# kazuto1011/dusty-gan

Measured on AMD Instinct MI355X. Metric: G+D train images/sec on 64x1024 LiDAR (steps/sec beside it), higher is better.
Workload: dtype bf16

## Files before the change

dusty_gan_amd/csrc/api.hip:

```cpp
#include "common.h"
#include "thin.h"

int dg_conv_direct_launch(const ConvP* p, hipStream_t stream);
int dg_lrelu_bits_launch(const ConvP* p, hipStream_t stream);
int dg_conv_mfma_launch(const ConvP* p, hipStream_t stream, int force, int fp32x3, int wg_cap, DgConvPlan* plan);
int dg_wgrad_mfma_dma_supported(const WgradP* p);
int dg_wgrad_mfma_dma_launch(const WgradP* p, int accumulate, int pairs, hipStream_t stream, DgWgradPlan* plan);
int dg_wgrad_mfma_dma_group_launch(const WgradP* items, int n, int pairs, int rounds, hipStream_t stream, DgWgradPlan* plans);
int dg_proj_stream_supported(const ConvP* p);
int dg_proj_stream_launch(const ConvP* p, hipStream_t stream, DgConvPlan* plan);
int dg_wgrad_mfma_ws_splits(const WgradP* p, int accumulate);
int dg_wgrad_direct_ws_splits(const WgradP* p);
int dg_wgrad_direct_launch(const WgradP* p, hipStream_t stream);
int dg_wgrad_mfma_launch(const WgradP* p, int accumulate, hipStream_t stream, int x3);

namespace {

enum ConvKernel { CONV_DIRECT, CONV_THIN, CONV_MFMA, CONV_PROJ_STREAM };

int select_conv(const DgConv* p, int force_flags, ConvKernel* k, ThinConvPick* thin, DgConvPlan* plan) {
  if (p && (p->mask_out || p->mask_in)) {
    if (p->mask_out && p->epi != EPI_LRELU) return DG_EINVAL;
    if (p->mask_in && p->epi != EPI_MASK) return DG_EINVAL;
    if (p->out_sn != 1 || p->N % 8 != 0 || p->out_sp % 8 != 0 || p->out_sb % 8 != 0) return DG_EUNSUPPORTED;
  }
  if (!p || !p->in || !p->out || !p->w) return DG_EINVAL;
  if (p->B <= 0 || p->K <= 0 || p->N <= 0) return DG_EINVAL;
  if (p->mode != MODE_GEMM && (p->Hc < 2 || p->Wc < 2)) return DG_EINVAL;
  if (p->epi == EPI_MASK && !p->aux) return DG_EINVAL;
  if (p->bias && p->bias_mod <= 0) return DG_EINVAL;
  if (p->dbias && p->bias_mod <= 0) return DG_EINVAL;
  if (plan) *plan = DgConvPlan{};
  const int force = force_flags & ~DG_FORCE_FP32X3;
  const bool mfma_ok = !p->nscale && dg_conv_mfma_supported(p), thin_ok = thin_conv_pick(p, thin) == DG_OK;
  const bool proj_ok = dg_proj_stream_supported(p);
  bool ok = true;
  if (force == DG_FORCE_AUTO) *k = proj_ok ? CONV_PROJ_STREAM : (mfma_ok ? CONV_MFMA : (thin_ok ? CONV_THIN : CONV_DIRECT));
  else if (force == DG_FORCE_PROJ_STREAM) *k = CONV_PROJ_STREAM, ok = proj_ok;
  else if (force == DG_FORCE_MFMA || force == DG_FORCE_LOCKSTEP || force == DG_FORCE_PINGPONG ||
           force == DG_FORCE_PINGPONG_SINGLE) *k = CONV_MFMA, ok = mfma_ok;
  else if (force == DG_FORCE_THIN) *k = CONV_THIN, ok = thin_ok;
  else *k = CONV_DIRECT;
  return ok ? DG_OK : DG_EUNSUPPORTED;
}

int conv_run(const DgConv* p, ConvKernel k, const ThinConvPick& thin, int force_flags, int wg_cap, hipStream_t s, DgConvPlan* plan) {
  if (k == CONV_PROJ_STREAM) return dg_proj_stream_launch(p, s, plan);
  if (k == CONV_MFMA)
    return dg_conv_mfma_launch(p, s, force_flags & ~DG_FORCE_FP32X3, (force_flags & DG_FORCE_FP32X3) ? 1 : 0, wg_cap, plan);
  if (!plan) return k == CONV_THIN ? thin_conv_launch(p, thin, s) : dg_conv_direct_launch(p, s);
  plan->family = k == CONV_THIN ? DG_CONV_FAMILY_THIN : DG_CONV_FAMILY_DIRECT;
  if (k == CONV_THIN)
    plan->thin_mfma = thin.thin_mfma, plan->mask_bits = thin.mask_bits, plan->dbias_rows = thin.dbias_rows, plan->sum_parts = thin.sum_parts;
  return DG_OK;
}

int conv_dispatch(const DgConv* p, int force_flags, int wg_cap, hipStream_t s, DgConvPlan* plan) {
  ConvKernel k;
  ThinConvPick thin;
  int rc = select_conv(p, force_flags, &k, &thin, plan);
  if (rc || plan || !p->mask_out) return rc ? rc : conv_run(p, k, thin, force_flags, wg_cap, s, plan);
  DgConvPlan pl{};
  rc = conv_run(p, k, thin, force_flags, wg_cap, nullptr, &pl);
  if (rc == DG_OK) rc = conv_run(p, k, thin, force_flags, wg_cap, s, nullptr);
// ... 2 lines not shown
}

struct WgradKernel {
  int variant;
  int pairs;
  int splits;
  long ws_floats;
  bool takes_gmod;
  bool zero_dw;
  ThinWgradPick thin;
};

int select_wgrad(const DgWgrad* p, int accumulate, int force_flags, WgradKernel* k) {
  if (!p || !p->a || !p->g || !p->dw) return DG_EINVAL;
  if (p->B <= 0 || p->Ci <= 0 || p->Co <= 0 || p->Hc <= 0 || p->Wc <= 0) return DG_EINVAL;
  const int force = force_flags & ~DG_FORCE_FP32X3;
  ThinWgradPick thin;
  const bool mfma_ok = dg_wgrad_mfma_supported(p), thin_ok = thin_wgrad_pick(p, &thin) == DG_OK;
  const bool pairs = force == DG_FORCE_WG_DMA_PAIRS || force == DG_FORCE_WG_DMA_NOPAIRS;
  *k = WgradKernel{};
  if ((force == DG_FORCE_AUTO || force == DG_FORCE_MFMA || pairs) && mfma_ok && dg_wgrad_mfma_dma_supported(p)) {
    k->variant = DG_WGRAD_VARIANT_DMA, k->takes_gmod = true;
    k->pairs = force == DG_FORCE_WG_DMA_PAIRS ? 1 : (force == DG_FORCE_WG_DMA_NOPAIRS ? 2 : 0);
    return DG_OK;
  }
  if (force == DG_FORCE_AUTO)
    k->variant = mfma_ok ? DG_WGRAD_VARIANT_MFMA : (thin_ok ? DG_WGRAD_VARIANT_THIN : DG_WGRAD_VARIANT_DIRECT);
  else if (force == DG_FORCE_MFMA || force == DG_FORCE_WG_REGSTAGED) k->variant = mfma_ok ? DG_WGRAD_VARIANT_MFMA : 0;
  else if (force == DG_FORCE_THIN) k->variant = thin_ok ? DG_WGRAD_VARIANT_THIN : 0;
  else if (!pairs) k->variant = DG_WGRAD_VARIANT_DIRECT;
  if (!k->variant) return DG_EUNSUPPORTED;
// ... 74 lines not shown
```

dusty_gan_amd/csrc/conv_mfma.hip:

```cpp
#include "mfma_common.h"

#ifndef DG_CONV_SETPRIO
#define DG_CONV_SETPRIO 1
#endif

template <typename T, int BM, int BN, int SB, int NS, bool X3 = false>
__global__ __launch_bounds__(256, 2) void conv_mfma_kernel(ConvP p, int tiles_n, int tiles_x, int dbg) {
  static_assert(!X3 || sizeof(T) == 4, "fp32x3: fp32 operands");
  constexpr int ES = sizeof(T);
  constexpr bool PRIO = DG_CONV_SETPRIO;
  constexpr int BK = SB / ES;
  constexpr int EPC = 16 / ES;
  constexpr int TM = BM / 64, TN = BN / 64;
  constexpr int RPI = 1024 / SB;
  constexpr int CPR = SB / 16;
  constexpr int KS = SB / 32;
  constexpr int STAGE = (BM + BN) * SB;
  constexpr int IA = BM / RPI / 4, IB = BN / RPI / 4;
  constexpr int IPT = IA + IB;
  __shared__ __attribute__((aligned(1024))) unsigned char lds[NS * STAGE];

  const int nwg = gridDim.x, id = blockIdx.x;
  const int q8 = nwg >> 3, r8 = nwg & 7, xcd = id & 7;
  const int logical = (xcd < r8 ? xcd * (q8 + 1) : r8 * (q8 + 1) + (xcd - r8) * q8) + (id >> 3);
// ... 289 lines not shown
  conv_mfma_kernel<T, BM, BN, 128, 2, X3><<<(unsigned)nwg, 256, 0, stream>>>(*p, tiles_n, tiles_x, 0);
  HIP_CHECK_RET(hipGetLastError());
  return DG_OK;
}

template <typename T, bool X3 = false>
static int launch_tiles(const ConvP* p, hipStream_t stream, DgConvPlan* plan) {
  const bool m128 = p->mode == MODE_GEMM ? false : (p->Wc % 128 == 0);
  const bool n128 = p->N % 128 == 0;
  if (m128 && n128) return launch_cfg<T, 128, 128, X3>(p, stream, plan);
  if (m128) return launch_cfg<T, 128, 64, X3>(p, stream, plan);
  if (n128) return launch_cfg<T, 64, 128, X3>(p, stream, plan);
  return launch_cfg<T, 64, 64, X3>(p, stream, plan);
}

int dg_conv_mfma_pp_launch(const ConvP* p, hipStream_t stream, int min_tiles, int wg_cap, DgConvPlan* plan, int dual);

extern "C" int dg_conv_mfma_supported(const ConvP* p) {
  if (p->in_dtype == DG_BF16X2 || p->out_dtype == DG_BF16X2 || p->w_dtype == DG_BF16X2) {
    DgConvPlan pl;
    return dg_conv_mfma_pp_launch(p, nullptr, 1, 0, &pl, 1) == DG_OK;
  }
  const int es = p->in_dtype == DG_BF16 ? 2 : 4;
  const int BK = 128 / es;
  if (p->in_dtype != p->out_dtype || p->in_dtype != p->w_dtype) return 0;
  if (p->K % BK != 0 || p->N % 64 != 0) return 0;
  if (p->in_sk != 1 || p->w_sk != 1 || p->out_sn != 1) return 0;
  if (p->mode == MODE_GEMM) return p->dbias == nullptr;
  if (!p->ring) return 0;
  if (p->Wc % 64 != 0) return 0;
  if (p->dbias && p->bias_mod < p->N) return 0;
  return 1;
}

int dg_conv_mfma_persist_launch_bf16(const ConvP* p, hipStream_t stream, int auto_rule, int wg_cap, DgConvPlan* plan);
int dg_conv_mfma_persist_launch_f32(const ConvP* p, hipStream_t stream, int auto_rule, int wg_cap, DgConvPlan* plan);

int dg_conv_mfma_launch(const ConvP* p, hipStream_t stream, int force, int fp32x3, int wg_cap, DgConvPlan* plan) {
  if (!dg_conv_mfma_supported(p)) return DG_EUNSUPPORTED;
  if (force == DG_FORCE_PINGPONG || force == DG_FORCE_PINGPONG_SINGLE)
    return (p->in_dtype == DG_BF16 || p->in_dtype == DG_BF16X2)
               ? dg_conv_mfma_pp_launch(p, stream, 1, wg_cap, plan, force == DG_FORCE_PINGPONG) : DG_EUNSUPPORTED;
  if (force == DG_FORCE_LOCKSTEP) {
    if (p->in_dtype == DG_BF16X2) return DG_EUNSUPPORTED;
    return p->in_dtype == DG_BF16 ? dg_conv_mfma_persist_launch_bf16(p, stream, 0, wg_cap, plan)
                                  : dg_conv_mfma_persist_launch_f32(p, stream, 0, wg_cap, plan);
  }
  if (p->in_dtype == DG_BF16X2) return dg_conv_mfma_pp_launch(p, stream, 1, wg_cap, plan, 1);
  if (p->in_dtype == DG_BF16) {
    const int rc = dg_conv_mfma_pp_launch(p, stream, 256, wg_cap, plan, 1);
    if (rc != DG_EUNSUPPORTED) return rc;
  }
  const bool x3 = p->in_dtype == DG_F32 && fp32x3;
  if (!x3) {
    const int rc = p->in_dtype == DG_BF16 ? dg_conv_mfma_persist_launch_bf16(p, stream, 1, wg_cap, plan)
                                          : dg_conv_mfma_persist_launch_f32(p, stream, 1, wg_cap, plan);
    if (rc != DG_EUNSUPPORTED) return rc;
  }
  if (x3) return launch_tiles<float, true>(p, stream, plan);
  return p->in_dtype == DG_BF16 ? launch_tiles<bf16>(p, stream, plan) : launch_tiles<float>(p, stream, plan);
}
```

dusty_gan_amd/csrc/conv_mfma_persist_impl.h:

```cpp
#pragma once
#include "mfma_common.h"

namespace persist {

template <typename T> struct StageWrite;
template <> struct StageWrite<bf16> {
  static __device__ __forceinline__ void put(unsigned addr, float v) {
    const bf16 h = (bf16)v;
    const unsigned bits = (unsigned)__builtin_bit_cast(unsigned short, h);
    asm volatile("ds_write_b16 %0, %1" ::"v"(addr), "v"(bits) : "memory");
  }
};
template <> struct StageWrite<float> {
  static __device__ __forceinline__ void put(unsigned addr, float v) {
    asm volatile("ds_write_b32 %0, %1" ::"v"(addr), "v"(v) : "memory");
  }
};

struct Tile {
  int nt, xt, px, Y, bt;
};

template <int MODE>
__device__ __forceinline__ bool next_tile(Tile& t, int tiles_n, int tiles_x, int rows) {
// ... 18 lines not shown
    int r, ky;
    if (dg_tap1d(MODE, adj, 0, Y, Hc, i, r, ky)) {
      list |= (unsigned long long)((r << 2) | ky) << (10 * n);
      ++n;
    }
  }
  return n;
}

#define DG_WAITV(n) asm volatile("s_waitcnt vmcnt(%0)" ::"n"(n) : "memory")

struct Geo {
  int tiles_n, tiles_x, ntiles;
  int SW, NSB, lsw;
  int dbg;
};

template <typename T, int BM, int BN, int WM, int WN, int SB, int NS, int MODE>
__global__ __launch_bounds__(64 * WM * WN, 1) void conv_kernel(ConvP p, Geo g) {
  constexpr int NWV = WM * WN;
  constexpr int ES = sizeof(T);
  constexpr int BK = SB / ES;
  constexpr int EPC = 16 / ES;
  constexpr int TM = BM / WM / 32, TN = BN / WN / 32;
  constexpr int RPI = 1024 / SB;
  constexpr int CPR = SB / 16;
  constexpr int KS = SB / 32;
  constexpr int STAGE = (BM + BN) * SB;
  constexpr int IA = BM / RPI / NWV, IB = BN / RPI / NWV;
  constexpr int IPT = IA + IB;
// ... 424 lines not shown
```

dusty_gan_amd/csrc/conv_mfma_pp.hip:

```cpp
#include "conv_mfma_persist_impl.h"

#include <type_traits>

namespace pp {

using persist::Geo;
using persist::Tile;

typedef __attribute__((ext_vector_type(4))) float f32x4_t;

#define PP_WAIT(vm) asm volatile("s_waitcnt vmcnt(%0) lgkmcnt(0)" ::"n"(vm) : "memory")

constexpr int NHT = 256;
struct HTab { unsigned long long e[NHT]; };

__device__ __forceinline__ unsigned long long pp_stamp() {
  unsigned long long t;
  __builtin_amdgcn_sched_barrier(0);
  asm volatile("s_memtime %0\n\ts_waitcnt lgkmcnt(0)" : "=s"(t)::"memory");
  __builtin_amdgcn_sched_barrier(0);
  return t;
}

template <int CTRL>
__device__ __forceinline__ float row_add(float v) {
  const int s = __builtin_amdgcn_update_dpp(0, __builtin_bit_cast(int, v), CTRL, 0xf, 0xf, false);
  return v + __builtin_bit_cast(float, s);
}

template <int BN, int MODE, bool MASK, bool DUAL = false, bool BITS = false, bool X2 = false>
__global__ __launch_bounds__(512, 2) void conv_pp_kernel(ConvP p, Geo g, HTab ht) {
  static_assert(MASK || !BITS, "BITS: a flavour of the EPI_MASK epilogue");
  static_assert(!X2 || !BITS, "X2: mask source = the saved activation's hi half");
  static_assert(!DUAL || (MODE == MODE_UP && BN == 128), "DUAL: both column parities of a 64-channel MODE_UP layer");
  constexpr int NCH = DUAL ? BN / 2 : BN;
  constexpr int BM = 256, NWV = 8, WN = 2;
  constexpr int SB = 128;
  constexpr int WC = BN / WN;
  constexpr int TM = 4, TN = WC / 16;
  constexpr int CPL = 4 * TN;
  constexpr int IMG_ROWS = 264;
  constexpr int AIMG = IMG_ROWS * SB;
  constexpr int BT = BN * SB;
  constexpr int PSTAGE = AIMG + 2 * BT;
  constexpr int NPS = 2;
  constexpr int IA = 4, IB = BN / 8 / NWV;
  constexpr int NST = TM * CPL * 2 / 16;
// ... 11 lines not shown
  constexpr int dbg = DG_PP_DIAG;
#else
  constexpr int dbg = 0;
#endif

  const int G = gridDim.x;
  const int q8 = G >> 3, r8 = G & 7, xcd = blockIdx.x & 7;
  const int gi0 = xcd < r8 ? xcd * (q8 + 1) : r8 * (q8 + 1) + (xcd - r8) * q8;
  const int nwx = q8 + (xcd < r8 ? 1 : 0);
  const int tq = g.ntiles / G, tr = g.ntiles % G;
  const int xs = gi0 * tq + (gi0 < tr ? gi0 : tr);
  const int xe = (gi0 + nwx) * tq + (gi0 + nwx < tr ? gi0 + nwx : tr);
  const int t0 = xs + (int)(blockIdx.x >> 3);
  const int tcount = t0 < xe ? (xe - t0 + nwx - 1) / nwx : 0;
  if (tcount == 0) {
    if (MASK && p.dbias && p.dbias_part)
      for (int n = threadIdx.x; n < p.N; n += 64 * NWV) p.dbias_part[(long)blockIdx.x * p.N + n] = 0.f;
    return;
  }

  const unsigned long long tk0 = (dbg & 8) ? pp_stamp() : 0ull;
  const unsigned long long tr0 = (dbg & 8) ? __builtin_amdgcn_s_memrealtime() : 0ull;
  const int tid = threadIdx.x;
  const int wave = __builtin_amdgcn_readfirstlane(tid >> 6), lane = tid & 63;
  const int KC = p.K / 64;
  const int Ws = MODE == MODE_S2 ? 2 * p.Wc : p.Wc, cmul = MODE == MODE_S2 ? 2 : 1;
  const int Wo = MODE == MODE_S2 ? p.Wc : 2 * p.Wc;
  const int rows = MODE == MODE_S2 ? p.Hc : 2 * p.Hc;
  const int tiles_n = g.tiles_n, tiles_x = g.tiles_x;

  auto tile_at = [&](int t) {
// ... 17 lines not shown
    dstep.xt = r % tiles_x; r /= tiles_x;
    dstep.px = 0;
    if (MODE == MODE_UP && !DUAL) { dstep.px = r & 1; r >>= 1; }
    dstep.Y = r % rows; dstep.bt = r / rows;
    dstep.nt = __builtin_amdgcn_readfirstlane(dstep.nt); dstep.xt = __builtin_amdgcn_readfirstlane(dstep.xt);
    dstep.px = __builtin_amdgcn_readfirstlane(dstep.px); dstep.Y = __builtin_amdgcn_readfirstlane(dstep.Y);
    dstep.bt = __builtin_amdgcn_readfirstlane(dstep.bt);
  }
  auto tile_next = [&](Tile& t) __attribute__((always_inline)) {
    int c;
    t.nt += dstep.nt; c = t.nt >= tiles_n; if (c) t.nt -= tiles_n;
    t.xt += dstep.xt + c; c = t.xt >= tiles_x; if (c) t.xt -= tiles_x;
    if (MODE == MODE_UP && !DUAL) { t.px += dstep.px + c; c = t.px >> 1; t.px &= 1; }
    t.Y += dstep.Y + c; c = t.Y >= rows; if (c) t.Y -= rows;
    t.bt += dstep.bt + c;
  };

  const bf16* in = (const bf16*)p.in;
  const bf16* w = (const bf16*)p.w;
  const int lrow = lane >> 3, pos = lane & 7;
  auto swzA = [](int row) { return ((row >> 1) & 3) << 1; };
  auto swzB = [](int row) { return ((row >> 1) & 1) | (((row / CPL) & 3) << 1); };

  unsigned voffA[NPAIR][IA + 1], voffB[IB];
  int colA[IA + 1];
  unsigned sampA[IA + 1];
  {
    const int pitch = g.SW + (DUAL ? 2 : 1);
#pragma unroll
    for (int u = 0; u <= IA; ++u) {
// ... 96 lines not shown
      for (int i = 0; i < TM; ++i) {
        const char* src = mb + (long)i * px_b;
        if (CPL == 16) asm volatile("global_load_ushort %0, %1, %2" : "=v"(mbits[i]) : "v"(pix_off_m), "s"(src) : "memory");
        else asm volatile("global_load_ubyte %0, %1, %2" : "=v"(mbits[i]) : "v"(pix_off_m), "s"(src) : "memory");
      }
    } else {
      const char* ab = (const char*)((const bf16*)p.aux + tile_off(t));
#pragma unroll
      for (int i = 0; i < TM; ++i) {
        const char* src = ab + (long)(i * 16) * px_b;
        asm volatile("global_load_dwordx4 %0, %1, %2" : "=v"(axr[(NST / TM) * i]) : "v"(pix_off), "s"(src) : "memory");
        if (NST / TM == 2) asm volatile("global_load_dwordx4 %0, %1, %2 offset:16" : "=v"(axr[2 * i + 1]) : "v"(pix_off), "s"(src) : "memory");
      }
    }
  };
  auto flush_db = [&](float (&dbacc)[CPL], int nt) __attribute__((always_inline)) {
#pragma unroll
    for (int c = 0; c < CPL; ++c) dbacc[c] = row_add<0xB1>(dbacc[c]);
#pragma unroll
    for (int c = 0; c < CPL; ++c) dbacc[c] = row_add<0x4E>(dbacc[c]);
#pragma unroll
    for (int c = 0; c < CPL; ++c) dbacc[c] = row_add<0x124>(dbacc[c]);
#pragma unroll
    for (int c = 0; c < CPL; ++c) dbacc[c] = row_add<0x128>(dbacc[c]);
    if (a16 == 0) {
      const unsigned ad = sdbw0 + (unsigned)(nt * NCH * 4) + lane_c0 * 4;
#pragma unroll
      for (int c = 0; c < CPL; ++c) asm volatile("ds_add_f32 %0, %1 offset:%2" ::"v"(ad), "v"(dbacc[c]), "n"(c * 4) : "memory");
    }
  };
  auto epilogue = [&](const Tile& t) __attribute__((always_inline)) {
    char* ob = (char*)(out + tile_off(t));
    if (MASK && !BITS) {
#pragma unroll
      for (int i = 0; i < NST; ++i) asm volatile("" : "+v"(axr[i]));
    }
    if (BITS) {
#pragma unroll
      for (int i = 0; i < TM; ++i) asm volatile("" : "+v"(mbits[i]));
// ... 100 lines not shown
          }
          continue;
        }
        if (h == 0 && i > 0) store_row(i - 1);
        asm volatile("ds_write_b128 %0, %1" ::"v"(scr_w ^ (unsigned)(h << 4)), "v"(pk) : "memory");
      }
      if (STRIP) {
        asm volatile("s_waitcnt lgkmcnt(0)" ::: "memory");
#pragma unroll
        for (int h = 0; h < NRD; ++h)
          asm volatile("ds_read_b128 %0, %1 offset:%2" : "=v"(rd[h]) : "v"(scr_r), "n"(h * 1024) : "memory");
      }
      __builtin_amdgcn_sched_barrier(0);
    }
    if (STRIP) store_row(TM - 1);
    if (want_db) flush_db(dbacc, t.nt);
    zero_acc();
  };

  const bool stamps = (dbg & 8) != 0;
  unsigned long long tsum[6] = {0, 0, 0, 0, 0, 0};
  unsigned long long tend = 0, tkf = 0;

  if (wave >= 4) __builtin_amdgcn_s_barrier();
  unsigned so_c = PSTAGE, so_i = 0;
  bool pending = false;
  bool warm = true;
  Tile tprev = first;
  const long tap_b = (long)p.w_st * 2;
  const unsigned spb = (unsigned)p.in_sp * 2u;

// ... 94 lines not shown
      if (stamps) t4 = pp_stamp();
      if (ISS || t == 0 || wave < 4) __builtin_amdgcn_s_barrier();
      if (stamps) {
        t5 = pp_stamp();
        tsum[0] += t1 - t0; tsum[1] += t2 - t1; tsum[2] += t3 - t2; tsum[3] += t4 - t3; tsum[4] += t5 - t4;
        tend = t5;
      }
    };
    step(std::integral_constant<int, 0>{});
    step(std::integral_constant<int, 1>{});
    const unsigned sw_ = so_c; so_c = so_i; so_i = sw_;
  };

  Tile ti = first;
  for (int c = 0; c < tcount; ++c) {
    unsigned long long hl;
    int nh;
    {
      const unsigned long long e = ht.e[ti.Y];
      nh = (int)(e >> 60) & 7;
      hl = e & 0x0fffffffffffffffull;
    }
    const char* in_t = (const char*)(in + (long)(ti.bt * g.NSB) * p.in_sb);
    const char* w_t = (const char*)(w + (long)(ti.nt * NCH) * p.w_sn);
    const int x0 = cmul * ti.xt * BM;
#pragma unroll
    for (int pi = 0; pi < NPAIR; ++pi) {
      const int cb = MODE == MODE_S2 ? pi - 1 : ((DUAL || ti.px == 0) ? -1 : 0);
#pragma unroll
      for (int u = 0; u <= IA; ++u)
// ... 7 lines not shown
      const char* sA_row = in_t + (long)it_r * Ws * spb;
      const char* sB_row = w_t + (long)(it_ky * 4) * tap_b;
      for (int kc = 0; kc < (X2 ? 3 : 1) * KC; ++kc) {
        const int kq = X2 ? kc / 3 : kc, sub = X2 ? kc - 3 * kq : 0;
        const char* sA_k = sA_row + kq * (X2 ? 2 * SB : SB) + (sub == 1 ? SB : 0);
        const char* sB_k = sB_row + kq * (X2 ? 2 * SB : SB) + (sub == 2 ? SB : 0);
#pragma unroll
        for (int pi = 0; pi < NPAIR; ++pi) {
          pair_iter(std::true_type{}, firstg, pi, sA_k, sB_k + (long)(kxa + pi) * tap_b, sB_k + (long)(kxb + pi) * tap_b,
                    sB_k + 2 * tap_b, sB_k);
          if (firstg) { firstg = false; warm = false; }
        }
      }
    }
    tprev = ti;
    tile_next(ti);
  }
  pair_iter(std::false_type{}, true, 0, nullptr, nullptr, nullptr, nullptr, nullptr);
  const unsigned long long tk2 = (dbg & 8) ? pp_stamp() : 0ull;
  const unsigned long long tr2 = (dbg & 8) ? __builtin_amdgcn_s_memrealtime() : 0ull;
  if (pending && !(dbg & 4)) {
    asm volatile("s_waitcnt vmcnt(0)" ::: "memory");
    epilogue(tprev);
  }
  if (stamps && blockIdx.x == 0 && lane == 0) {
    float* sink = (float*)p.out + wave * 8;
    asm volatile("s_waitcnt vmcnt(0)" ::: "memory");
    const unsigned long long tk3 = pp_stamp();
    for (int k = 0; k < 6; ++k) sink[k] = (float)tsum[k];
    float* ph = (float*)p.out + 64 + wave * 8;
    ph[0] = (float)(tk1 - tk0); ph[1] = (float)(tkf - tk0); ph[2] = (float)(tk2 - tk0); ph[3] = (float)(tk3 - tk0);
    ph[4] = (float)tcount;
    ph[5] = (float)(tr2 - tr0);
  }
  if (want_db) {
    asm volatile("s_waitcnt vmcnt(0) lgkmcnt(0)" ::: "memory");
    __syncthreads();
    for (int n = tid; n < p.N; n += 64 * NWV) {
      float v;
      if (db_rows) {
        v = s_bias[n];
#pragma unroll
        for (int r = 1; r < DBW; ++r) v += s_bias[r * p.N + n];
      } else v = s_db[n];
      if (p.dbias_part) p.dbias_part[(long)blockIdx.x * p.N + n] = v;
      else atomicAdd(&p.dbias[n % p.bias_mod], v);
    }
  }
}

template <int BN, int MODE, bool MASK, bool DUAL = false, bool X2 = false>
int launch(const ConvP* p, const Geo& g0, hipStream_t stream, int wg_cap, DgConvPlan* plan) {
  constexpr int CPL_ = (BN / 2 / 16) * 4;
  const bool bits_ok = !X2 && p->out_sn == 1 && p->out_sb % 8 == 0 && p->out_sp % CPL_ == 0 && p->N % CPL_ == 0;
  if (!MASK && p->mask_out && !bits_ok) return DG_EUNSUPPORTED;
  const bool bits = MASK && p->mask_in && bits_ok;
  Geo g = g0;
  static int resident = 0;
  if (!resident) {
    int dev = 0, cus = 0;
    HIP_CHECK_RET(hipGetDevice(&dev));
    HIP_CHECK_RET(hipDeviceGetAttribute(&cus, hipDeviceAttributeMultiprocessorCount, dev));
    resident = cus;
  }
  g.dbg = 0;
  const int cap = (wg_cap > 0 && wg_cap < resident) ? wg_cap : resident;
  const int G = g.ntiles < cap ? g.ntiles : cap;
  if (plan) {
    plan->family = DG_CONV_FAMILY_PINGPONG; plan->bm = DUAL ? 512 : 256; plan->bn = DUAL ? BN / 2 : BN; plan->tiles = g.ntiles; plan->workgroups = G;
    plan->tiles_per_wg = (g.ntiles + G - 1) / G;
    plan->mask_bits = MASK ? (bits ? 2 : 0) : 1;
    plan->dbias_rows = (MASK && (DUAL ? 8 : 4) * p->N <= 2048) ? G : 0;
    return DG_OK;
  }
  HTab ht;
  {
    const int rows = MODE == MODE_S2 ? p->Hc : 2 * p->Hc;
    for (int y = 0; y < NHT; ++y) {
      unsigned long long hl = 0;
      const int nh = y < rows ? persist::pack_htaps<MODE>(p->adj, y, p->Hc, hl) : 0;
      ht.e[y] = hl | ((unsigned long long)nh << 60);
    }
  }
  if constexpr (X2) {
    conv_pp_kernel<BN, MODE, MASK, DUAL, false, true><<<(unsigned)G, 512, 0, stream>>>(*p, g, ht);
  } else if constexpr (MASK) {
    if (bits) conv_pp_kernel<BN, MODE, true, DUAL, true><<<(unsigned)G, 512, 0, stream>>>(*p, g, ht);
    else conv_pp_kernel<BN, MODE, true, DUAL, false><<<(unsigned)G, 512, 0, stream>>>(*p, g, ht);
  } else conv_pp_kernel<BN, MODE, false, DUAL><<<(unsigned)G, 512, 0, stream>>>(*p, g, ht);
  HIP_CHECK_RET(hipGetLastError());
  return DG_OK;
}

}

int dg_conv_mfma_pp_launch(const ConvP* p0, hipStream_t stream, int min_tiles, int wg_cap, DgConvPlan* plan, int dual) {
  if (p0->mode != MODE_S2 && p0->mode != MODE_UP) return DG_EUNSUPPORTED;
  const bool x2 = p0->in_dtype == DG_BF16X2;
  if (p0->in_dtype != p0->out_dtype || p0->in_dtype != p0->w_dtype || (p0->in_dtype != DG_BF16 && !x2)) return DG_EUNSUPPORTED;
  ConvP q = *p0;
  if (x2) {
    if (p0->K % 64 || p0->N % 64 || p0->in_sp % 64 || p0->in_sb % 64 || p0->out_sp % 64 || p0->out_sb % 64 || p0->w_sn % 64 ||
        p0->w_st % 64 || (((size_t)p0->in | (size_t)p0->out | (size_t)p0->w | (size_t)p0->aux) & 255))
      return DG_EUNSUPPORTED;
    if (p0->mask_out || p0->mask_in) return DG_EUNSUPPORTED;
    q.in_sb *= 2; q.in_sp *= 2; q.out_sb *= 2; q.out_sp *= 2; q.w_st *= 2; q.w_sn *= 2;
  }
  const ConvP* p = &q;
  if (p->K % 64 != 0 || !p->ring || p->nscale) return DG_EUNSUPPORTED;
  if (p->mode == MODE_UP && p->adj && p->K < 128) return DG_EUNSUPPORTED;
  if (p->in_sk != 1 || p->w_sk != 1 || p->out_sn != 1) return DG_EUNSUPPORTED;
  if (p->out_sp % 8 != 0 || p->in_sp % 8 != 0 || p->w_sn % 8 != 0) return DG_EUNSUPPORTED;
  if (p->N > 512 || (p->bias && p->bias_mod < p->N && p->N % p->bias_mod != 0)) return DG_EUNSUPPORTED;
  if (p->dbias && p->bias_mod < p->N) return DG_EUNSUPPORTED;
  const int Ws = p->mode == MODE_S2 ? 2 * p->Wc : p->Wc;
  if ((Ws & (Ws - 1)) != 0 || p->in_sp * 2 >= (1 << 24)) return DG_EUNSUPPORTED;
  if ((p->mode == MODE_S2 ? p->Hc : 2 * p->Hc) > 256) return DG_EUNSUPPORTED;
  const bool mask = p->epi == EPI_MASK;
  if (mask ? p->bias != nullptr : p->dbias != nullptr) return DG_EUNSUPPORTED;
  if (p->rowscale && p->B > 512) return DG_EUNSUPPORTED;
  persist::Geo g;
  int bn = 0;
  if (dual && p->mode == MODE_UP && p->N % 128 != 0 && p->N % 64 == 0 && persist::make_geo<256, 64>(p, g) && g.SW >= 64 &&
      g.NSB * (g.SW + 2) <= 264 && g.ntiles / 2 >= min_tiles) {
    g.ntiles /= 2;
    if (x2) return mask ? pp::launch<128, MODE_UP, true, true, true>(p, g, stream, wg_cap, plan)
                        : pp::launch<128, MODE_UP, false, true, true>(p, g, stream, wg_cap, plan);
    return mask ? pp::launch<128, MODE_UP, true, true>(p, g, stream, wg_cap, plan)
                : pp::launch<128, MODE_UP, false, true>(p, g, stream, wg_cap, plan);
  }
  if (p->N % 128 == 0 && persist::make_geo<256, 128>(p, g) && g.SW >= 64 && g.ntiles >= min_tiles) bn = 128;
  else if (p->N % 64 == 0 && persist::make_geo<256, 64>(p, g) && g.SW >= 64 && g.ntiles >= min_tiles) bn = 64;
  if (!bn) return DG_EUNSUPPORTED;
  const int sel = (bn == 128 ? 0 : 4) + (p->mode == MODE_UP ? 2 : 0) + (mask ? 1 : 0);
  if (x2) switch (sel) {
    case 0: return pp::launch<128, MODE_S2, false, false, true>(p, g, stream, wg_cap, plan);
    case 1: return pp::launch<128, MODE_S2, true, false, true>(p, g, stream, wg_cap, plan);
    case 2: return pp::launch<128, MODE_UP, false, false, true>(p, g, stream, wg_cap, plan);
    case 3: return pp::launch<128, MODE_UP, true, false, true>(p, g, stream, wg_cap, plan);
    case 4: return pp::launch<64, MODE_S2, false, false, true>(p, g, stream, wg_cap, plan);
    case 5: return pp::launch<64, MODE_S2, true, false, true>(p, g, stream, wg_cap, plan);
    case 6: return pp::launch<64, MODE_UP, false, false, true>(p, g, stream, wg_cap, plan);
    default: return pp::launch<64, MODE_UP, true, false, true>(p, g, stream, wg_cap, plan);
  }
  switch (sel) {
    case 0: return pp::launch<128, MODE_S2, false>(p, g, stream, wg_cap, plan);
    case 1: return pp::launch<128, MODE_S2, true>(p, g, stream, wg_cap, plan);
    case 2: return pp::launch<128, MODE_UP, false>(p, g, stream, wg_cap, plan);
    case 3: return pp::launch<128, MODE_UP, true>(p, g, stream, wg_cap, plan);
    case 4: return pp::launch<64, MODE_S2, false>(p, g, stream, wg_cap, plan);
    case 5: return pp::launch<64, MODE_S2, true>(p, g, stream, wg_cap, plan);
    case 6: return pp::launch<64, MODE_UP, false>(p, g, stream, wg_cap, plan);
    default: return pp::launch<64, MODE_UP, true>(p, g, stream, wg_cap, plan);
  }
}
```

dusty_gan_amd/engine.py:

```python
import ctypes as C
import math
import os
import warnings
from collections import OrderedDict, namedtuple

import torch

from . import _lib as L

ARCH_ID = {"none": 0, "dusty1": 1, "dusty2": 2}

PROFILE = None
TRACE = None


def _align(n, a=64):
    return (n + a - 1) // a * a


class Segment:
    __slots__ = ("name", "off", "shape", "numel", "kind")

    def __init__(self, name, off, shape, kind):
        self.name, self.off, self.shape, self.kind = name, off, tuple(shape), kind
# ... 587 lines not shown
            ws = Ops._dbias_ws.get(str(x.device))
            if ws is None:
                ws = Ops._dbias_ws[str(x.device)] = torch.zeros(L.DBIAS_WS_FLOATS, dtype=torch.float32, device=x.device)
            p.dbias_ws = L.ptr(ws)
        final = None

        def plan():
            nonlocal final
            if final is None:
                final = self._conv_plan(p)
            return final
        db_rows = 0
        if dbias is not None and DETERMINISTIC:
            pl = plan()
            if pl.dbias_rows > 0:
                part = WGRAD_WS.take(pl.dbias_rows * N, x.device)
                if part is not None:
                    db_rows, p.dbias_part = pl.dbias_rows, part
        if TRACE is not None:
            pl = plan()
            TRACE.append(("conv", pl.family, pl.bm, pl.bn, pl.tiles, pl.workgroups, pl.tiles_per_wg, _conv_tag(p), pl.thin_mfma,
                          (1 if p.mask_out else 0) | (pl.mask_bits & 2 if p.mask_in else 0)))

        def record():
            pl = plan()
            names = {L.DG_CONV_FAMILY_THIN: "conv_thin_kernel", L.DG_CONV_FAMILY_DIRECT: "conv_direct_kernel"}
            mb = 0
            if p.mask_out or p.mask_in:
                mb = pl.mask_bits if p.mask_in else 1
            cost = conv_algorithmic(mode, B, Hc, Wc, K, N, ies, oes, _es(p.w_dtype), epi == L.EPI_MASK, mb)
            return (names.get(pl.family, "conv_mfma_kernel"),) + cost + (_conv_tag(p),)
# ... 767 lines not shown
```

include/dusty_gan_hip.h:

```cpp
#ifndef DUSTY_GAN_HIP_H
#define DUSTY_GAN_HIP_H
#include <stdint.h>

#ifdef __cplusplus
extern "C" {
#endif

#define DG_OK 0
#define DG_EINVAL 1
#define DG_EUNSUPPORTED 2
#define DG_EHIP 3

#define DG_F32 0
#define DG_BF16 1
#define DG_BF16X2 2

#define DG_MODE_S2 0
#define DG_MODE_UP 1
#define DG_MODE_GEMM 2

#define DG_EPI_LINEAR 0
#define DG_EPI_LRELU 1
#define DG_EPI_MASK 2

// ... 44 lines not shown
} DgWgrad;

int dg_conv(const DgConv* p, int force, void* stream);
#define DG_FORCE_AUTO 0
#define DG_FORCE_DIRECT 1
#define DG_FORCE_MFMA 2
#define DG_FORCE_THIN 3
#define DG_FORCE_LOCKSTEP 4
#define DG_FORCE_PINGPONG 5
#define DG_FORCE_WG_REGSTAGED 6
#define DG_FORCE_WG_DMA_PAIRS 7
#define DG_FORCE_WG_DMA_NOPAIRS 8
#define DG_FORCE_PINGPONG_SINGLE 9
#define DG_FORCE_PROJ_STREAM 10
#define DG_FORCE_FP32X3 0x100
#define DG_CONV_FAMILY_DIRECT 1
#define DG_CONV_FAMILY_MFMA 2
#define DG_CONV_FAMILY_THIN 3
#define DG_CONV_FAMILY_LOCKSTEP 4
#define DG_CONV_FAMILY_PINGPONG 5
#define DG_CONV_FAMILY_PROJ_STREAM 6
typedef struct DgConvPlan {
  int family;
  int bm, bn;
  int tiles;
  int workgroups;
  int tiles_per_wg;
  int thin_mfma;
  int mask_bits;
  int dbias_rows;
  int sum_parts;
} DgConvPlan;
int dg_conv_ex(const DgConv* p, int force, int wg_cap, void* stream);
int dg_conv_plan(const DgConv* p, int force, int wg_cap, DgConvPlan* plan);
int dg_conv_mfma_supported(const DgConv* p);

int dg_wgrad(const DgWgrad* p, int accumulate, int force, void* stream);
#define DG_WGRAD_VARIANT_DIRECT 1
#define DG_WGRAD_VARIANT_MFMA 2
#define DG_WGRAD_VARIANT_THIN 3
#define DG_WGRAD_VARIANT_DMA 5
#define DG_WGRAD_VARIANT_THIN_MFMA 7
typedef struct DgWgradPlan {
  int variant;
  int splits;
  long ws_floats;
// ... 324 lines not shown
```

Baseline: 13690.

## Balance per-workgroup tap load in ping-pong conv by flipping edge rows across batches

Edge rows have fewer vertical taps, so some workgroups in the persistent ping-pong conv get less work than others. The host now searches a small set of flip shifts and picks the one that swaps edge-row indices for alternating batch groups to minimise the worst per-workgroup tap count. That choice is cached and passed to a new FLIP kernel variant. Because flipping breaks the per-workgroup deterministic bias-gradient reduction, the FLIP path writes per-tile bias partials to extra workspace slots and runs a second reduction kernel. This adds a launch and extra workspace in exchange for better load balance.

```diff
diff --git a/dusty_gan_amd/csrc/api.hip b/dusty_gan_amd/csrc/api.hip
--- a/dusty_gan_amd/csrc/api.hip
+++ b/dusty_gan_amd/csrc/api.hip
@@ -3,7 +3,7 @@
 
 int dg_conv_direct_launch(const ConvP* p, hipStream_t stream);
 int dg_lrelu_bits_launch(const ConvP* p, hipStream_t stream);
-int dg_conv_mfma_launch(const ConvP* p, hipStream_t stream, int force, int fp32x3, int wg_cap, DgConvPlan* plan);
+int dg_conv_mfma_launch(const ConvP* p, hipStream_t stream, int force, int fp32x3, int rowflip, int wg_cap, DgConvPlan* plan);
 int dg_wgrad_mfma_dma_supported(const WgradP* p);
 int dg_wgrad_mfma_dma_launch(const WgradP* p, int accumulate, int pairs, hipStream_t stream, DgWgradPlan* plan);
 int dg_wgrad_mfma_dma_group_launch(const WgradP* items, int n, int pairs, int rounds, hipStream_t stream, DgWgradPlan* plans);
@@ -15,6 +15,9 @@
 int dg_wgrad_mfma_launch(const WgradP* p, int accumulate, hipStream_t stream, int x3);
 
 namespace {
+
+constexpr int ROWFLIP_FLAGS = DG_FORCEFLAG_NO_ROWFLIP | DG_FORCEFLAG_ROWFLIP_MASK;
+constexpr int FORCE_FLAGS = DG_FORCE_FP32X3 | ROWFLIP_FLAGS;
 
 enum ConvKernel { CONV_DIRECT, CONV_THIN, CONV_MFMA, CONV_PROJ_STREAM };
 
@@ -31,7 +34,7 @@
   if (p->bias && p->bias_mod <= 0) return DG_EINVAL;
   if (p->dbias && p->bias_mod <= 0) return DG_EINVAL;
   if (plan) *plan = DgConvPlan{};
-  const int force = force_flags & ~DG_FORCE_FP32X3;
+  const int force = force_flags & ~FORCE_FLAGS;
   const bool mfma_ok = !p->nscale && dg_conv_mfma_supported(p), thin_ok = thin_conv_pick(p, thin) == DG_OK;
   const bool proj_ok = dg_proj_stream_supported(p);
   bool ok = true;
@@ -47,7 +50,8 @@
 int conv_run(const DgConv* p, ConvKernel k, const ThinConvPick& thin, int force_flags, int wg_cap, hipStream_t s, DgConvPlan* plan) {
   if (k == CONV_PROJ_STREAM) return dg_proj_stream_launch(p, s, plan);
   if (k == CONV_MFMA)
-    return dg_conv_mfma_launch(p, s, force_flags & ~DG_FORCE_FP32X3, (force_flags & DG_FORCE_FP32X3) ? 1 : 0, wg_cap, plan);
+    return dg_conv_mfma_launch(p, s, force_flags & ~FORCE_FLAGS, (force_flags & DG_FORCE_FP32X3) ? 1 : 0,
+                               force_flags & ROWFLIP_FLAGS, wg_cap, plan);
   if (!plan) return k == CONV_THIN ? thin_conv_launch(p, thin, s) : dg_conv_direct_launch(p, s);
   plan->family = k == CONV_THIN ? DG_CONV_FAMILY_THIN : DG_CONV_FAMILY_DIRECT;
   if (k == CONV_THIN)
@@ -80,7 +84,7 @@
 int select_wgrad(const DgWgrad* p, int accumulate, int force_flags, WgradKernel* k) {
   if (!p || !p->a || !p->g || !p->dw) return DG_EINVAL;
   if (p->B <= 0 || p->Ci <= 0 || p->Co <= 0 || p->Hc <= 0 || p->Wc <= 0) return DG_EINVAL;
-  const int force = force_flags & ~DG_FORCE_FP32X3;
+  const int force = force_flags & ~FORCE_FLAGS;
   ThinWgradPick thin;
   const bool mfma_ok = dg_wgrad_mfma_supported(p), thin_ok = thin_wgrad_pick(p, &thin) == DG_OK;
   const bool pairs = force == DG_FORCE_WG_DMA_PAIRS || force == DG_FORCE_WG_DMA_NOPAIRS;
diff --git a/dusty_gan_amd/csrc/conv_mfma.hip b/dusty_gan_amd/csrc/conv_mfma.hip
--- a/dusty_gan_amd/csrc/conv_mfma.hip
+++ b/dusty_gan_amd/csrc/conv_mfma.hip
@@ -327,12 +327,12 @@
   return launch_cfg<T, 64, 64, X3>(p, stream, plan);
 }
 
-int dg_conv_mfma_pp_launch(const ConvP* p, hipStream_t stream, int min_tiles, int wg_cap, DgConvPlan* plan, int dual);
+int dg_conv_mfma_pp_launch(const ConvP* p, hipStream_t stream, int min_tiles, int wg_cap, DgConvPlan* plan, int dual, int rowflip);
 
 extern "C" int dg_conv_mfma_supported(const ConvP* p) {
   if (p->in_dtype == DG_BF16X2 || p->out_dtype == DG_BF16X2 || p->w_dtype == DG_BF16X2) {
     DgConvPlan pl;
-    return dg_conv_mfma_pp_launch(p, nullptr, 1, 0, &pl, 1) == DG_OK;
+    return dg_conv_mfma_pp_launch(p, nullptr, 1, 0, &pl, 1, 0) == DG_OK;
   }
   const int es = p->in_dtype == DG_BF16 ? 2 : 4;
   const int BK = 128 / es;
@@ -349,19 +349,19 @@
 int dg_conv_mfma_persist_launch_bf16(const ConvP* p, hipStream_t stream, int auto_rule, int wg_cap, DgConvPlan* plan);
 int dg_conv_mfma_persist_launch_f32(const ConvP* p, hipStream_t stream, int auto_rule, int wg_cap, DgConvPlan* plan);
 
-int dg_conv_mfma_launch(const ConvP* p, hipStream_t stream, int force, int fp32x3, int wg_cap, DgConvPlan* plan) {
+int dg_conv_mfma_launch(const ConvP* p, hipStream_t stream, int force, int fp32x3, int rowflip, int wg_cap, DgConvPlan* plan) {
   if (!dg_conv_mfma_supported(p)) return DG_EUNSUPPORTED;
   if (force == DG_FORCE_PINGPONG || force == DG_FORCE_PINGPONG_SINGLE)
     return (p->in_dtype == DG_BF16 || p->in_dtype == DG_BF16X2)
-               ? dg_conv_mfma_pp_launch(p, stream, 1, wg_cap, plan, force == DG_FORCE_PINGPONG) : DG_EUNSUPPORTED;
+               ? dg_conv_mfma_pp_launch(p, stream, 1, wg_cap, plan, force == DG_FORCE_PINGPONG, rowflip) : DG_EUNSUPPORTED;
   if (force == DG_FORCE_LOCKSTEP) {
     if (p->in_dtype == DG_BF16X2) return DG_EUNSUPPORTED;
     return p->in_dtype == DG_BF16 ? dg_conv_mfma_persist_launch_bf16(p, stream, 0, wg_cap, plan)
                                   : dg_conv_mfma_persist_launch_f32(p, stream, 0, wg_cap, plan);
   }
-  if (p->in_dtype == DG_BF16X2) return dg_conv_mfma_pp_launch(p, stream, 1, wg_cap, plan, 1);
+  if (p->in_dtype == DG_BF16X2) return dg_conv_mfma_pp_launch(p, stream, 1, wg_cap, plan, 1, rowflip);
   if (p->in_dtype == DG_BF16) {
-    const int rc = dg_conv_mfma_pp_launch(p, stream, 256, wg_cap, plan, 1);
+    const int rc = dg_conv_mfma_pp_launch(p, stream, 256, wg_cap, plan, 1, rowflip);
     if (rc != DG_EUNSUPPORTED) return rc;
   }
   const bool x3 = p->in_dtype == DG_F32 && fp32x3;
diff --git a/dusty_gan_amd/csrc/conv_mfma_persist_impl.h b/dusty_gan_amd/csrc/conv_mfma_persist_impl.h
--- a/dusty_gan_amd/csrc/conv_mfma_persist_impl.h
+++ b/dusty_gan_amd/csrc/conv_mfma_persist_impl.h
@@ -56,6 +56,7 @@
   int tiles_n, tiles_x, ntiles;
   int SW, NSB, lsw;
   int dbg;
+  int flip_shift = -1;
 };
 
 template <typename T, int BM, int BN, int WM, int WN, int SB, int NS, int MODE>
diff --git a/dusty_gan_amd/csrc/conv_mfma_pp.hip b/dusty_gan_amd/csrc/conv_mfma_pp.hip
--- a/dusty_gan_amd/csrc/conv_mfma_pp.hip
+++ b/dusty_gan_amd/csrc/conv_mfma_pp.hip
@@ -1,5 +1,8 @@
 #include "conv_mfma_persist_impl.h"
 
+#include <algorithm>
+#include <map>
+#include <mutex>
 #include <type_traits>
 
 namespace pp {
@@ -28,9 +31,10 @@
   return v + __builtin_bit_cast(float, s);
 }
 
-template <int BN, int MODE, bool MASK, bool DUAL = false, bool BITS = false, bool X2 = false>
+template <int BN, int MODE, bool MASK, bool DUAL = false, bool BITS = false, bool X2 = false, bool FLIP = false>
 __global__ __launch_bounds__(512, 2) void conv_pp_kernel(ConvP p, Geo g, HTab ht) {
   static_assert(MASK || !BITS, "BITS: a flavour of the EPI_MASK epilogue");
+  static_assert(MASK || !FLIP, "FLIP: compiled into the EPI_MASK flavour only");
   static_assert(!X2 || !BITS, "X2: mask source = the saved activation's hi half");
   static_assert(!DUAL || (MODE == MODE_UP && BN == 128), "DUAL: both column parities of a 64-channel MODE_UP layer");
   constexpr int NCH = DUAL ? BN / 2 : BN;
@@ -72,7 +76,7 @@
   const int t0 = xs + (int)(blockIdx.x >> 3);
   const int tcount = t0 < xe ? (xe - t0 + nwx - 1) / nwx : 0;
   if (tcount == 0) {
-    if (MASK && p.dbias && p.dbias_part)
+    if (MASK && !FLIP && p.dbias && p.dbias_part)
       for (int n = threadIdx.x; n < p.N; n += 64 * NWV) p.dbias_part[(long)blockIdx.x * p.N + n] = 0.f;
     return;
   }
@@ -120,6 +124,11 @@
     if (MODE == MODE_UP && !DUAL) { t.px += dstep.px + c; c = t.px >> 1; t.px &= 1; }
     t.Y += dstep.Y + c; c = t.Y >= rows; if (c) t.Y -= rows;
     t.bt += dstep.bt + c;
+  };
+  auto flip_row = [&](Tile& t) __attribute__((always_inline)) {
+    if constexpr (!FLIP) return;
+    const int edge = (t.Y < 2 || t.Y >= rows - 2) ? 1 : 0;
+    t.Y ^= (t.bt >> g.flip_shift) & edge;
   };
 
   const bf16* in = (const bf16*)p.in;
@@ -246,7 +255,8 @@
       }
     }
   };
-  auto flush_db = [&](float (&dbacc)[CPL], int nt) __attribute__((always_inline)) {
+  auto flush_db = [&](float (&dbacc)[CPL], const Tile& td) __attribute__((always_inline)) {
+    const int nt = td.nt;
 #pragma unroll
     for (int c = 0; c < CPL; ++c) dbacc[c] = row_add<0xB1>(dbacc[c]);
 #pragma unroll
@@ -255,6 +265,15 @@
     for (int c = 0; c < CPL; ++c) dbacc[c] = row_add<0x124>(dbacc[c]);
 #pragma unroll
     for (int c = 0; c < CPL; ++c) dbacc[c] = row_add<0x128>(dbacc[c]);
+    if constexpr (FLIP) {
+      if (a16 == 0 && p.dbias_part) {
+        const int tlin = ((((td.bt * rows + td.Y) * ((MODE == MODE_UP && !DUAL) ? 2 : 1) + td.px) * tiles_x + td.xt) * tiles_n) + td.nt;
+        float* dst = p.dbias_part + (long)gridDim.x * p.N + ((long)tlin * DBW + (DUAL ? wave : wave / WN)) * NCH + lane_c0;
+#pragma unroll
+        for (int c = 0; c < CPL; ++c) dst[c] = dbacc[c];
+      }
+      return;
+    }
     if (a16 == 0) {
       const unsigned ad = sdbw0 + (unsigned)(nt * NCH * 4) + lane_c0 * 4;
 #pragma unroll
@@ -385,7 +404,7 @@
       __builtin_amdgcn_sched_barrier(0);
     }
     if (STRIP) store_row(TM - 1);
-    if (want_db) flush_db(dbacc, t.nt);
+    if (want_db) flush_db(dbacc, t);
     zero_acc();
   };
 
@@ -510,6 +529,7 @@
 
   Tile ti = first;
   for (int c = 0; c < tcount; ++c) {
+    flip_row(ti);
     unsigned long long hl;
     int nh;
     {
@@ -547,6 +567,7 @@
       }
     }
     tprev = ti;
+    flip_row(ti);
     tile_next(ti);
   }
   pair_iter(std::false_type{}, true, 0, nullptr, nullptr, nullptr, nullptr, nullptr);
@@ -566,7 +587,7 @@
     ph[4] = (float)tcount;
     ph[5] = (float)(tr2 - tr0);
   }
-  if (want_db) {
+  if (want_db && !FLIP) {
     asm volatile("s_waitcnt vmcnt(0) lgkmcnt(0)" ::: "memory");
     __syncthreads();
     for (int n = tid; n < p.N; n += 64 * NWV) {
@@ -582,8 +603,99 @@
   }
 }
 
+template <int NCH, int DBW>
+__global__ __launch_bounds__(256) void dbias_rows_kernel(float* part, int N, int ntiles, int tiles_n) {
+  const int G = gridDim.x;
+  const int q8 = G >> 3, r8 = G & 7, xcd = blockIdx.x & 7;
+  const int gi0 = xcd < r8 ? xcd * (q8 + 1) : r8 * (q8 + 1) + (xcd - r8) * q8;
+  const int nwx = q8 + (xcd < r8 ? 1 : 0);
+  const int tq = ntiles / G, tr = ntiles % G;
+  const int xs = gi0 * tq + (gi0 < tr ? gi0 : tr);
+  const int xe = (gi0 + nwx) * tq + (gi0 + nwx < tr ? gi0 + nwx : tr);
+  const int t0 = xs + (int)(blockIdx.x >> 3);
+  float* slots = part + (long)G * N;
+  for (int n = threadIdx.x; n < N; n += 256) {
+    const int nt = n / NCH, ch = n - nt * NCH;
+    float row[DBW];
+#pragma unroll
+    for (int r = 0; r < DBW; ++r) row[r] = 0.f;
+    for (int t = t0; t < xe; t += nwx) {
+      if (t % tiles_n != nt) continue;
+      float* src = slots + (long)t * DBW * NCH + ch;
+#pragma unroll
+      for (int r = 0; r < DBW; ++r) {
+        row[r] += src[r * NCH];
+      }
+    }
+    float v = row[0];
+#pragma unroll
+    for (int r = 1; r < DBW; ++r) v += row[r];
+    part[(long)blockIdx.x * N + n] = v;
+  }
+}
+
+struct RowSched {
+  int flip_shift, htaps_max, htaps_total;
+};
+inline int rows_walk_max(int ntiles, int G, int tiles_n, int tiles_x, int npar, int rows, const int* nh, int shift) {
+  const int q8 = G >> 3, r8 = G & 7, tq = ntiles / G, tr = ntiles % G;
+  int worst = 0;
+  for (int xcd = 0; xcd < 8; ++xcd) {
+    const int gi0 = xcd < r8 ? xcd * (q8 + 1) : r8 * (q8 + 1) + (xcd - r8) * q8;
+    const int nwx = q8 + (xcd < r8 ? 1 : 0);
+    const int xs = gi0 * tq + (gi0 < tr ? gi0 : tr);
+    const int xe = (gi0 + nwx) * tq + (gi0 + nwx < tr ? gi0 + nwx : tr);
+    for (int j = 0; j < nwx; ++j) {
+      int sum = 0;
+      for (int t = xs + j; t < xe; t += nwx) {
+        const int mt = t / tiles_n / tiles_x / npar;
+        const int Y = mt % rows, bt = mt / rows;
+        const int edge = (Y < 2 || Y >= rows - 2) ? 1 : 0;
+        sum += nh[shift >= 0 ? Y ^ ((bt >> shift) & edge) : Y];
+      }
+      if (sum > worst) worst = sum;
+    }
+  }
+  return worst;
+}
+inline RowSched rows_sched(int ntiles, int G, int tiles_n, int tiles_x, int npar, int rows, int mode, int adj, int Hc, int req) {
+  struct Key {
+    int v[10];
+    bool operator<(const Key& o) const { return std::lexicographical_compare(v, v + 10, o.v, o.v + 10); }
+  };
+  static std::mutex mu;
+  static std::map<Key, RowSched> cache;
+  const bool off = (req & DG_FORCEFLAG_NO_ROWFLIP) != 0;
+  const int forced = off ? -1 : (req & DG_FORCEFLAG_ROWFLIP_MASK) / DG_FORCEFLAG_ROWFLIP_UNIT - 1;
+  const Key key{{ntiles, G, tiles_n, tiles_x, npar, rows, mode, adj, Hc, req}};
+  std::lock_guard<std::mutex> lock(mu);
+  const auto it = cache.find(key);
+  if (it != cache.end()) return it->second;
+  int nh[NHT];
+  RowSched r{-1, 0, 0};
+  for (int y = 0; y < rows; ++y) {
+    nh[y] = 0;
+    for (int i = 0, src, ky; i < 6; ++i) nh[y] += dg_tap1d(mode, adj, 0, y, Hc, i, src, ky) ? 1 : 0;
+    r.htaps_total += nh[y];
+  }
+  const long total = (long)r.htaps_total * (ntiles / rows);
+  r.htaps_total = total < 0x7fffffffL ? (int)total : 0x7fffffff;
+  r.htaps_max = rows_walk_max(ntiles, G, tiles_n, tiles_x, npar, rows, nh, -1);
+  const bool can = adj && rows % 2 == 0;
+  if (can && forced >= 0) {
+    r.flip_shift = forced;
+    r.htaps_max = rows_walk_max(ntiles, G, tiles_n, tiles_x, npar, rows, nh, forced);
+  } else if (can && !off)
+    for (int s = 0; s <= 3; ++s) {
+      const int m = rows_walk_max(ntiles, G, tiles_n, tiles_x, npar, rows, nh, s);
+      if (m < r.htaps_max) r.htaps_max = m, r.flip_shift = s;
+    }
+  if (cache.size() < 4096) cache[key] = r;
+  return r;
+}
+
 template <int BN, int MODE, bool MASK, bool DUAL = false, bool X2 = false>
-int launch(const ConvP* p, const Geo& g0, hipStream_t stream, int wg_cap, DgConvPlan* plan) {
+int launch(const ConvP* p, const Geo& g0, hipStream_t stream, int wg_cap, DgConvPlan* plan, int rowflip) {
   constexpr int CPL_ = (BN / 2 / 16) * 4;
   const bool bits_ok = !X2 && p->out_sn == 1 && p->out_sb % 8 == 0 && p->out_sp % CPL_ == 0 && p->N % CPL_ == 0;
   if (!MASK && p->mask_out && !bits_ok) return DG_EUNSUPPORTED;
@@ -599,35 +711,52 @@
   g.dbg = 0;
   const int cap = (wg_cap > 0 && wg_cap < resident) ? wg_cap : resident;
   const int G = g.ntiles < cap ? g.ntiles : cap;
+  const int rows = MODE == MODE_S2 ? p->Hc : 2 * p->Hc;
+  constexpr int DBW_ = DUAL ? 8 : 4;
+  const bool db_rows = MASK && DBW_ * p->N <= 2048;
+  const bool may_flip = MASK && !X2 && db_rows && (plan || !p->dbias || p->dbias_part);
+  const RowSched rs = rows_sched(g.ntiles, G, g.tiles_n, g.tiles_x, (MODE == MODE_UP && !DUAL) ? 2 : 1, rows, MODE, p->adj ? 1 : 0,
+                                 p->Hc, may_flip ? rowflip : DG_FORCEFLAG_NO_ROWFLIP);
+  g.flip_shift = rs.flip_shift;
+  const int db_extra = rs.flip_shift >= 0 ? g.ntiles / g.tiles_n * DBW_ : 0;
   if (plan) {
+    plan->htaps_max = rs.htaps_max; plan->htaps_total = rs.htaps_total;
     plan->family = DG_CONV_FAMILY_PINGPONG; plan->bm = DUAL ? 512 : 256; plan->bn = DUAL ? BN / 2 : BN; plan->tiles = g.ntiles; plan->workgroups = G;
     plan->tiles_per_wg = (g.ntiles + G - 1) / G;
     plan->mask_bits = MASK ? (bits ? 2 : 0) : 1;
-    plan->dbias_rows = (MASK && (DUAL ? 8 : 4) * p->N <= 2048) ? G : 0;
+    plan->dbias_rows = db_rows ? G : 0;
+    plan->dbias_ws_rows = db_extra ? G + db_extra : 0;
     return DG_OK;
   }
   HTab ht;
-  {
-    const int rows = MODE == MODE_S2 ? p->Hc : 2 * p->Hc;
-    for (int y = 0; y < NHT; ++y) {
-      unsigned long long hl = 0;
-      const int nh = y < rows ? persist::pack_htaps<MODE>(p->adj, y, p->Hc, hl) : 0;
-      ht.e[y] = hl | ((unsigned long long)nh << 60);
-    }
-  }
-  if constexpr (X2) {
-    conv_pp_kernel<BN, MODE, MASK, DUAL, false, true><<<(unsigned)G, 512, 0, stream>>>(*p, g, ht);
-  } else if constexpr (MASK) {
-    if (bits) conv_pp_kernel<BN, MODE, true, DUAL, true><<<(unsigned)G, 512, 0, stream>>>(*p, g, ht);
-    else conv_pp_kernel<BN, MODE, true, DUAL, false><<<(unsigned)G, 512, 0, stream>>>(*p, g, ht);
-  } else conv_pp_kernel<BN, MODE, false, DUAL><<<(unsigned)G, 512, 0, stream>>>(*p, g, ht);
+  for (int y = 0; y < NHT; ++y) {
+    unsigned long long hl = 0;
+    const int nh = y < rows ? persist::pack_htaps<MODE>(p->adj, y, p->Hc, hl) : 0;
+    ht.e[y] = hl | ((unsigned long long)nh << 60);
+  }
+  auto go = [&](auto flip_tag) {
+    constexpr bool FLIP = decltype(flip_tag)::value;
+    if constexpr (X2) {
+      conv_pp_kernel<BN, MODE, MASK, DUAL, false, true><<<(unsigned)G, 512, 0, stream>>>(*p, g, ht);
+    } else if constexpr (MASK) {
+      if (bits) conv_pp_kernel<BN, MODE, true, DUAL, true, false, FLIP><<<(unsigned)G, 512, 0, stream>>>(*p, g, ht);
+      else conv_pp_kernel<BN, MODE, true, DUAL, false, false, FLIP><<<(unsigned)G, 512, 0, stream>>>(*p, g, ht);
+    } else conv_pp_kernel<BN, MODE, false, DUAL><<<(unsigned)G, 512, 0, stream>>>(*p, g, ht);
+  };
+  if constexpr (MASK && !X2) {
+    if (g.flip_shift >= 0) go(std::true_type{}); else go(std::false_type{});
+  } else go(std::false_type{});
   HIP_CHECK_RET(hipGetLastError());
+  if (g.flip_shift >= 0 && p->dbias && p->dbias_part) {
+    dbias_rows_kernel<DUAL ? BN / 2 : BN, DBW_><<<(unsigned)G, 256, 0, stream>>>(p->dbias_part, p->N, g.ntiles, g.tiles_n);
+    HIP_CHECK_RET(hipGetLastError());
+  }
   return DG_OK;
 }
 
 }
 
-int dg_conv_mfma_pp_launch(const ConvP* p0, hipStream_t stream, int min_tiles, int wg_cap, DgConvPlan* plan, int dual) {
+int dg_conv_mfma_pp_launch(const ConvP* p0, hipStream_t stream, int min_tiles, int wg_cap, DgConvPlan* plan, int dual, int rowflip) {
   if (p0->mode != MODE_S2 && p0->mode != MODE_UP) return DG_EUNSUPPORTED;
   const bool x2 = p0->in_dtype == DG_BF16X2;
   if (p0->in_dtype != p0->out_dtype || p0->in_dtype != p0->w_dtype || (p0->in_dtype != DG_BF16 && !x2)) return DG_EUNSUPPORTED;
@@ -657,33 +786,39 @@
   if (dual && p->mode == MODE_UP && p->N % 128 != 0 && p->N % 64 == 0 && persist::make_geo<256, 64>(p, g) && g.SW >= 64 &&
       g.NSB * (g.SW + 2) <= 264 && g.ntiles / 2 >= min_tiles) {
     g.ntiles /= 2;
-    if (x2) return mask ? pp::launch<128, MODE_UP, true, true, true>(p, g, stream, wg_cap, plan)
-                        : pp::launch<128, MODE_UP, false, true, true>(p, g, stream, wg_cap, plan);
-    return mask ? pp::launch<128, MODE_UP, true, true>(p, g, stream, wg_cap, plan)
-                : pp::launch<128, MODE_UP, false, true>(p, g, stream, wg_cap, plan);
+    if (x2) return mask ? pp::launch<128, MODE_UP, true, true, true>(p, g, stream, wg_cap, plan, rowflip)
+                        : pp::launch<128, MODE_UP, false, true, true>(p, g, stream, wg_cap, plan, rowflip);
+    return mask ? pp::launch<128, MODE_UP, true, true>(p, g, stream, wg_cap, plan, rowflip)
+                : pp::launch<128, MODE_UP, false, true>(p, g, stream, wg_cap, plan, rowflip);
   }
   if (p->N % 128 == 0 && persist::make_geo<256, 128>(p, g) && g.SW >= 64 && g.ntiles >= min_tiles) bn = 128;
   else if (p->N % 64 == 0 && persist::make_geo<256, 64>(p, g) && g.SW >= 64 && g.ntiles >= min_tiles) bn = 64;
+#ifdef DG_PP_ADJ_N64
+  if (bn == 128 && p->adj && g.ntiles <= DG_PP_ADJ_N64) {
+    persist::Geo g64;
+    if (persist::make_geo<256, 64>(p, g64) && g64.SW >= 64) g = g64, bn = 64;
+  }
+#endif
   if (!bn) return DG_EUNSUPPORTED;
   const int sel = (bn == 128 ? 0 : 4) + (p->mode == MODE_UP ? 2 : 0) + (mask ? 1 : 0);
   if (x2) switch (sel) {
-    case 0: return pp::launch<128, MODE_S2, false, false, true>(p, g, stream, wg_cap, plan);
-    case 1: return pp::launch<128, MODE_S2, true, false, true>(p, g, stream, wg_cap, plan);
-    case 2: return pp::launch<128, MODE_UP, false, false, true>(p, g, stream, wg_cap, plan);
-    case 3: return pp::launch<128, MODE_UP, true, false, true>(p, g, stream, wg_cap, plan);
-    case 4: return pp::launch<64, MODE_S2, false, false, true>(p, g, stream, wg_cap, plan);
-    case 5: return pp::launch<64, MODE_S2, true, false, true>(p, g, stream, wg_cap, plan);
-    case 6: return pp::launch<64, MODE_UP, false, false, true>(p, g, stream, wg_cap, plan);
-    default: return pp::launch<64, MODE_UP, true, false, true>(p, g, stream, wg_cap, plan);
+    case 0: return pp::launch<128, MODE_S2, false, false, true>(p, g, stream, wg_cap, plan, rowflip);
+    case 1: return pp::launch<128, MODE_S2, true, false, true>(p, g, stream, wg_cap, plan, rowflip);
+    case 2: return pp::launch<128, MODE_UP, false, false, true>(p, g, stream, wg_cap, plan, rowflip);
+    case 3: return pp::launch<128, MODE_UP, true, false, true>(p, g, stream, wg_cap, plan, rowflip);
+    case 4: return pp::launch<64, MODE_S2, false, false, true>(p, g, stream, wg_cap, plan, rowflip);
+    case 5: return pp::launch<64, MODE_S2, true, false, true>(p, g, stream, wg_cap, plan, rowflip);
+    case 6: return pp::launch<64, MODE_UP, false, false, true>(p, g, stream, wg_cap, plan, rowflip);
+    default: return pp::launch<64, MODE_UP, true, false, true>(p, g, stream, wg_cap, plan, rowflip);
   }
   switch (sel) {
-    case 0: return pp::launch<128, MODE_S2, false>(p, g, stream, wg_cap, plan);
-    case 1: return pp::launch<128, MODE_S2, true>(p, g, stream, wg_cap, plan);
-    case 2: return pp::launch<128, MODE_UP, false>(p, g, stream, wg_cap, plan);
-    case 3: return pp::launch<128, MODE_UP, true>(p, g, stream, wg_cap, plan);
-    case 4: return pp::launch<64, MODE_S2, false>(p, g, stream, wg_cap, plan);
-    case 5: return pp::launch<64, MODE_S2, true>(p, g, stream, wg_cap, plan);
-    case 6: return pp::launch<64, MODE_UP, false>(p, g, stream, wg_cap, plan);
-    default: return pp::launch<64, MODE_UP, true>(p, g, stream, wg_cap, plan);
+    case 0: return pp::launch<128, MODE_S2, false>(p, g, stream, wg_cap, plan, rowflip);
+    case 1: return pp::launch<128, MODE_S2, true>(p, g, stream, wg_cap, plan, rowflip);
+    case 2: return pp::launch<128, MODE_UP, false>(p, g, stream, wg_cap, plan, rowflip);
+    case 3: return pp::launch<128, MODE_UP, true>(p, g, stream, wg_cap, plan, rowflip);
+    case 4: return pp::launch<64, MODE_S2, false>(p, g, stream, wg_cap, plan, rowflip);
+    case 5: return pp::launch<64, MODE_S2, true>(p, g, stream, wg_cap, plan, rowflip);
+    case 6: return pp::launch<64, MODE_UP, false>(p, g, stream, wg_cap, plan, rowflip);
+    default: return pp::launch<64, MODE_UP, true>(p, g, stream, wg_cap, plan, rowflip);
   }
 }
diff --git a/dusty_gan_amd/engine.py b/dusty_gan_amd/engine.py
--- a/dusty_gan_amd/engine.py
+++ b/dusty_gan_amd/engine.py
@@ -625,7 +625,7 @@
         if dbias is not None and DETERMINISTIC:
             pl = plan()
             if pl.dbias_rows > 0:
-                part = WGRAD_WS.take(pl.dbias_rows * N, x.device)
+                part = WGRAD_WS.take(max(pl.dbias_rows, pl.dbias_ws_rows) * N, x.device)
                 if part is not None:
                     db_rows, p.dbias_part = pl.dbias_rows, part
         if TRACE is not None:
diff --git a/include/dusty_gan_hip.h b/include/dusty_gan_hip.h
--- a/include/dusty_gan_hip.h
+++ b/include/dusty_gan_hip.h
@@ -82,6 +82,9 @@
 #define DG_FORCE_PINGPONG_SINGLE 9
 #define DG_FORCE_PROJ_STREAM 10
 #define DG_FORCE_FP32X3 0x100
+#define DG_FORCEFLAG_NO_ROWFLIP 0x200
+#define DG_FORCEFLAG_ROWFLIP_UNIT 0x400
+#define DG_FORCEFLAG_ROWFLIP_MASK 0x1c00
 #define DG_CONV_FAMILY_DIRECT 1
 #define DG_CONV_FAMILY_MFMA 2
 #define DG_CONV_FAMILY_THIN 3
@@ -98,6 +101,9 @@
   int mask_bits;
   int dbias_rows;
   int sum_parts;
+  int htaps_max;
+  int htaps_total;
+  int dbias_ws_rows;
 } DgConvPlan;
 int dg_conv_ex(const DgConv* p, int force, int wg_cap, void* stream);
 int dg_conv_plan(const DgConv* p, int force, int wg_cap, DgConvPlan* plan);
```

Result: no change. 13830, median of 6 (+1.0%).
